# eora-ai/torchok

Measured on AMD Instinct MI355X. Metric: images/sec (node) ResNet-50 224px bs256/GPU; step p50 ms, higher is better.
Workload: dtype bf16

## Files before the change

torchok_amd/csrc/gemm256.hip:

```cpp
#include "conv_common.h"
#include <stdlib.h>

namespace {

typedef __attribute__((address_space(3))) void lds_void;
typedef __attribute__((address_space(3))) char lds_char;

constexpr int GT = 256;
constexpr int GK = 64;
constexpr int TILE_B = GT * GK * 2;
constexpr int STAGE_B = 2 * TILE_B;
constexpr int NBLK = STAGE_B / 1024;
constexpr int NI = NBLK / 8;

__device__ __forceinline__ u32x4 lds_read16(uint32_t addr) {
  u32x4 v;
  asm volatile("ds_read_b128 %0, %1" : "=v"(v) : "v"(addr));
  return v;
}
__device__ __forceinline__ float row16_sum_f(float v) {
  v += __builtin_bit_cast(float, __builtin_amdgcn_update_dpp(0, __builtin_bit_cast(int, v), 0x128, 0xF, 0xF, false));
  v += __builtin_bit_cast(float, __builtin_amdgcn_update_dpp(0, __builtin_bit_cast(int, v), 0x124, 0xF, 0xF, false));
  v += __builtin_bit_cast(float, __builtin_amdgcn_update_dpp(0, __builtin_bit_cast(int, v), 0x122, 0xF, 0xF, false));
  v += __builtin_bit_cast(float, __builtin_amdgcn_update_dpp(0, __builtin_bit_cast(int, v), 0x121, 0xF, 0xF, false));
  return v;
}

template <int MODE>
__global__ __launch_bounds__(512, 1) void gemm256_kernel(ConvArgs a) {
  extern __shared__ __attribute__((aligned(16))) char smem[];
  const uint32_t lds_base = (uint32_t)(size_t)(lds_char*)smem;
  const int tid = threadIdx.x;
  const int lane = tid & 63;
  const int wave = __builtin_amdgcn_readfirstlane(tid >> 6);
  const int r = lane & 15, g = lane >> 4;
  const int wn = wave & 1, wm = wave >> 1;

  const int ntiles = a.gridM * a.gridN;
  const int KD = a.Ktot;
  const int KT = (KD + GK - 1) / GK;

  const __amdgpu_buffer_rsrc_t xsrd = __builtin_amdgcn_make_buffer_rsrc((void*)a.x, 0, a.x_bytes, 0x00020000);
  const __amdgpu_buffer_rsrc_t wsrd = __builtin_amdgcn_make_buffer_rsrc((void*)a.w, 0, a.w_bytes, 0x00020000);

  uint32_t voff[NI];
  int kq[NI];
#pragma unroll
  for (int j = 0; j < NI; ++j) {
    const int row = ((j * 8 + wave) & 31) * 8 + (lane >> 3);
    kq[j] = ((lane & 7) ^ ((row & 3) | (((row >> 3) & 1) << 2))) * 8;
  }
  auto setup = [&](int id, int& m0, int& n0) {
    const int mt = id / a.gridN, nt = id - mt * a.gridN;
    m0 = mt * GT;
    n0 = nt * GT;
#pragma unroll
    for (int j = 0; j < NI; ++j) {
      const int bid = j * 8 + wave;
      const int row = (bid & 31) * 8 + (lane >> 3);
      const bool isw = bid < 32;
      const int grow = (isw ? n0 : m0) + row;
      const bool ok = grow < (isw ? a.K : a.M);
      voff[j] = ok ? (uint32_t)(((long long)grow * KD + kq[j]) * 2) : 0xFFFFFFF0u;
    }
  };
  auto issue = [&](int kt, int buf, bool live) {
#pragma unroll
    for (int j = 0; j < NI; ++j) {
      const int bid = j * 8 + wave;
      uint32_t off = (live && voff[j] != 0xFFFFFFF0u && kt * GK + kq[j] < KD) ? voff[j] + (uint32_t)(kt * (GK * 2)) : 0xFFFFFFF0u;
      asm volatile("" : "+v"(off));
      lds_void* dst = (lds_void*)(smem + buf * STAGE_B + bid * 1024);
      if (bid < 32) __builtin_amdgcn_raw_ptr_buffer_load_lds(wsrd, dst, 16, off, 0, 0, 0);
      else __builtin_amdgcn_raw_ptr_buffer_load_lds(xsrd, dst, 16, off, 0, 0, 0);
    }
  };

  const uint32_t swz = (uint32_t)((r & 3) | (((r >> 2) & 1) << 2));
  const uint32_t swx = (uint32_t)((r & 3) | (((r >> 3) & 1) << 2));
  const uint32_t a_lane = (uint32_t)((wn * 128 + 8 * (r >> 2) + (r & 3)) * 128);
  const uint32_t b_lane = (uint32_t)(TILE_B + (wm * 64 + r) * 128);
  uint32_t a_ch[2], b_ch[2];
#pragma unroll
  for (int kk = 0; kk < 2; ++kk) {
    a_ch[kk] = (((uint32_t)(4 * kk + g)) ^ swz) << 4;
    b_ch[kk] = (((uint32_t)(4 * kk + g)) ^ swx) << 4;
  }

  int tile = tok_xcd_remap(blockIdx.x, gridDim.x);
  int m0, n0;
  setup(tile, m0, n0);
  int base = 0;
  issue(0, base, tile < ntiles);
  while (tile < ntiles) {
  f32x4 acc[4][2][4];
#pragma unroll
  for (int p = 0; p < 4; ++p)
#pragma unroll
    for (int b = 0; b < 2; ++b)
#pragma unroll
      for (int mb = 0; mb < 4; ++mb) acc[p][b][mb] = (f32x4){0.f, 0.f, 0.f, 0.f};
  for (int kt = 0; kt < KT; ++kt) {
    const int buf = (base + kt) & 1;
    asm volatile("s_waitcnt vmcnt(0)" ::: "memory");
    __builtin_amdgcn_s_barrier();
    issue(kt + 1, buf ^ 1, kt + 1 < KT);
    const uint32_t sb = lds_base + (uint32_t)(buf * STAGE_B);
#pragma unroll
    for (int kk = 0; kk < 2; ++kk) {
      u32x4 af[4][2], bfr[4];
#pragma unroll
      for (int mb = 0; mb < 4; ++mb) bfr[mb] = lds_read16(sb + b_lane + (uint32_t)(mb * 16 * 128) + b_ch[kk]);
#pragma unroll
      for (int p = 0; p < 4; ++p)
#pragma unroll
        for (int b = 0; b < 2; ++b) af[p][b] = lds_read16(sb + a_lane + (uint32_t)((32 * p + 4 * b) * 128) + a_ch[kk]);
      asm volatile("s_waitcnt lgkmcnt(0)" ::: "memory");
      __builtin_amdgcn_sched_barrier(0);
#pragma unroll
      for (int p = 0; p < 4; ++p)
#pragma unroll
        for (int b = 0; b < 2; ++b)
#pragma unroll
          for (int mb = 0; mb < 4; ++mb)
            acc[p][b][mb] = __builtin_amdgcn_mfma_f32_16x16x32_bf16(__builtin_bit_cast(bf16x8, af[p][b]),
                                                                    __builtin_bit_cast(bf16x8, bfr[mb]), acc[p][b][mb], 0, 0, 0);
    }
  }
  const int cm0 = m0, cn0 = n0, cmt = m0 / GT;
  const int next = tile + gridDim.x;
  base = (base + KT) & 1;
  if (next < ntiles) {
    setup(next, m0, n0);
    issue(0, base, true);
  }

  float s1[4][8], s2[4][8];
  if constexpr (MODE >= 1 && MODE <= 3) {
#pragma unroll
    for (int p = 0; p < 4; ++p)
#pragma unroll
      for (int e = 0; e < 8; ++e) { s1[p][e] = 0.f; s2[p][e] = 0.f; }
  }
#pragma unroll
  for (int p = 0; p < 4; ++p) {
    const int n8 = cn0 + wn * 128 + 32 * p + 8 * g;
    const bool nok = n8 + 8 <= a.K;
    float bv[8];
#pragma unroll
    for (int e = 0; e < 8; ++e) bv[e] = (a.bias != nullptr && nok) ? a.bias[n8 + e] : 0.f;
#pragma unroll
    for (int mb = 0; mb < 4; ++mb) {
      const int pix = cm0 + wm * 64 + 16 * mb + r;
      if (pix < a.M && nok) {
        const size_t off = (size_t)pix * a.K + n8;
        float v[8];
#pragma unroll
        for (int e = 0; e < 8; ++e) v[e] = acc[p][e >> 2][mb][e & 3] + bv[e];
        if (a.accumulate) {
          const bf16x8 old = ldg16(a.y + off);
#pragma unroll
          for (int e = 0; e < 8; ++e) v[e] += bf2f(old[e]);
        }
        bf16x8 o;
#pragma unroll
        for (int e = 0; e < 8; ++e) o[e] = f2bf(v[e]);
        if constexpr (MODE == 3) {
          const unsigned bits = (unsigned)a.bn_mask[off >> 3];
#pragma unroll
          for (int e = 0; e < 8; ++e) {
            if (!((bits >> e) & 1u)) o[e] = (bf16)0.f;
            s1[p][e] += bf2f(o[e]);
          }
        }
        stg16(a.y + off, o);
        if constexpr (MODE == 1) {
#pragma unroll
          for (int e = 0; e < 8; ++e) {
            const float q = bf2f(o[e]);
            s1[p][e] += q;
            s2[p][e] = fmaf(q, q, s2[p][e]);
          }
        }
        if constexpr (MODE == 2) {
          const bf16x8 yv = ldg16(a.bn_y + off);
          const unsigned bits = a.bn_mask != nullptr ? (unsigned)a.bn_mask[off >> 3] : 0xffu;
#pragma unroll
          for (int e = 0; e < 8; ++e) {
            const float dz = ((bits >> e) & 1u) ? bf2f(o[e]) : 0.f;
            s1[p][e] += dz;
            s2[p][e] = fmaf(dz, bf2f(yv[e]), s2[p][e]);
          }
        }
      }
    }
  }
  if constexpr (MODE >= 1 && MODE <= 3) {
    float* red = reinterpret_cast<float*>(smem + 2 * STAGE_B);
#pragma unroll
    for (int p = 0; p < 4; ++p)
#pragma unroll
      for (int e = 0; e < 8; ++e) {
        const float t1 = row16_sum_f(s1[p][e]), t2 = row16_sum_f(s2[p][e]);
        if (r == 15) {
          const int nl = wn * 128 + 32 * p + 8 * g + e;
          red[(0 * 4 + wm) * GT + nl] = t1;
          red[(1 * 4 + wm) * GT + nl] = t2;
        }
      }
    asm volatile("s_waitcnt lgkmcnt(0)" ::: "memory");
    __builtin_amdgcn_s_barrier();
    const int which = tid >> 8, c = tid & 255;
    const float t = red[(which * 4 + 0) * GT + c] + red[(which * 4 + 1) * GT + c] + red[(which * 4 + 2) * GT + c] +
                    red[(which * 4 + 3) * GT + c];
    const int n = cn0 + c;
    if (n < a.K) a.stats[((size_t)which * a.stat_rows + cmt) * a.K + n] = t;
    if (cmt == a.gridM - 1 && n < a.K)
      for (int rr = a.gridM; rr < a.stat_rows; ++rr) a.stats[((size_t)which * a.stat_rows + rr) * a.K + n] = 0.f;
    asm volatile("s_waitcnt lgkmcnt(0)" ::: "memory");
    __builtin_amdgcn_s_barrier();
  }
  tile = next;
  }
  asm volatile("s_waitcnt vmcnt(0) lgkmcnt(0)" ::: "memory");
}

int g256_flag() {
  static const int v = [] { const char* e = getenv("TOK_GEMM256"); return (int)(e ? atoi(e) : 1); }();
  return v;
}
int g256_min_k() {
  static const int v = [] { const char* e = getenv("TOK_GEMM256_MIN_K"); return (int)(e ? atoi(e) : 256); }();
  return v;
}
int g256_min_tiles() {
  static const int v = [] { const char* e = getenv("TOK_GEMM256_MIN_TILES"); return (int)(e ? atoi(e) : 128); }();
  return v;
}

}

bool gemm256_modes(const ConvArgs& a) {
  if (a.ep_scale != nullptr || a.sub != nullptr) return false;
  if (a.mask_store && (a.bn_mask == nullptr || a.stats == nullptr)) return false;
  if (a.y2 != nullptr || a.act_x != nullptr) return false;
  return true;
}
bool gemm256_serves(const ConvArgs& a) { return gemm256_geometry(a) && gemm256_modes(a); }

bool gemm256_geometry(const ConvArgs& a) {
  const int flag = g256_flag();
  if (!flag) return false;
  if (!(a.R == 1 && a.S == 1 && a.stride == 1 && a.pad == 0 && a.C != 4)) return false;
  if (a.Ktot % 8 != 0 || a.K % 8 != 0 || a.Ktot <= GK) return false;
  if (flag >= 3) return true;
  if (a.K < 192 || a.M < 4096) return false;
  const long long tiles = (long long)tok_cdiv(a.M, GT) * tok_cdiv(a.K, GT);
  const int nt = tok_cdiv(a.K, GT);
  if ((long long)nt * GT * 3 > (long long)a.K * 4) return false;
  if (tiles < g256_min_tiles()) return false;
  if (flag >= 2) return a.Ktot >= g256_min_k();
  return a.Ktot >= 384;
}

int gemm256_rows(const ConvArgs& a) { return (tok_cdiv(a.M, GT) + 7) / 8 * 8; }

void gemm256_tiles(const ConvArgs& a, int* gridM, int* gridN) { *gridM = tok_cdiv(a.M, GT); *gridN = tok_cdiv(a.K, GT); }
int gemm256_grid(int gridM, int gridN) { return gridM * gridN < 256 ? gridM * gridN : 256; }

int gemm256_launch(ConvArgs& a, hipStream_t st) {
  constexpr int smem = 2 * STAGE_B + 2 * 4 * GT * 4;
  const int grid = a.grid;
  if (a.mask_store) tok_launch_lds<&gemm256_kernel<3>>(smem, dim3(grid), dim3(512), smem, st, a);
  else if (a.stats == nullptr) tok_launch_lds<&gemm256_kernel<0>>(smem, dim3(grid), dim3(512), smem, st, a);
  else if (a.bn_y == nullptr) tok_launch_lds<&gemm256_kernel<1>>(smem, dim3(grid), dim3(512), smem, st, a);
  else tok_launch_lds<&gemm256_kernel<2>>(smem, dim3(grid), dim3(512), smem, st, a);
  return 0;
}
```

Before: 14520.

## Prefetch epilogue loads in groups and specialize accumulate path at compile time

Restructures the GEMM epilogue so the residual, bn_y and mask loads for a group of output column strips are issued ahead of time and overlap with the math and stores of the previous group. Rows and columns past the edge are clamped rather than branched on, so the loads and stores stay uniform. Bias is folded into the accumulators up front, and accumulate becomes a template parameter, which doubles the number of kernel instantiations. The prefetch buffers raise register pressure, which may spill at one wave per SIMD.

```diff
diff --git a/torchok_amd/csrc/gemm256.hip b/torchok_amd/csrc/gemm256.hip
--- a/torchok_amd/csrc/gemm256.hip
+++ b/torchok_amd/csrc/gemm256.hip
@@ -1,5 +1,6 @@
 #include "conv_common.h"
 #include <stdlib.h>
+#include <type_traits>
 
 namespace {
 
@@ -26,7 +27,7 @@
   return v;
 }
 
-template <int MODE>
+template <int MODE, bool ACC>
 __global__ __launch_bounds__(512, 1) void gemm256_kernel(ConvArgs a) {
   extern __shared__ __attribute__((aligned(16))) char smem[];
   const uint32_t lds_base = (uint32_t)(size_t)(lds_char*)smem;
@@ -142,57 +143,133 @@
 #pragma unroll
       for (int e = 0; e < 8; ++e) { s1[p][e] = 0.f; s2[p][e] = 0.f; }
   }
+  constexpr bool PRE_Y = MODE == 2, PRE_BITS = MODE == 2 || MODE == 3;
+  constexpr bool want_old = ACC;
+  const bool want_bits = PRE_BITS && (MODE == 3 || a.bn_mask != nullptr);
+  const bool want_bias = a.bias != nullptr;
+  const int strip0 = cm0 + wm * 64, cbase = cn0 + wn * 128;
+  const int strip0c = strip0 < a.M ? strip0 : a.M - 1;
+  const size_t sbase = (size_t)strip0c * a.K;
+  bf16* const yb = a.y + sbase;
+  const bf16* const bnb = a.bn_y + sbase;
+  const uint8_t* const mkb = a.bn_mask + (sbase >> 3);
+  uint32_t erow[4], ecol[4];
+  bool rok[4], nok[4];
+#pragma unroll
+  for (int mb = 0; mb < 4; ++mb) {
+    const int rr = 16 * mb + r, last = a.M - 1 - strip0c;
+    rok[mb] = strip0 + rr < a.M;
+    erow[mb] = (uint32_t)((rr < last ? rr : last) * a.K);
+  }
 #pragma unroll
   for (int p = 0; p < 4; ++p) {
-    const int n8 = cn0 + wn * 128 + 32 * p + 8 * g;
-    const bool nok = n8 + 8 <= a.K;
-    float bv[8];
-#pragma unroll
-    for (int e = 0; e < 8; ++e) bv[e] = (a.bias != nullptr && nok) ? a.bias[n8 + e] : 0.f;
-#pragma unroll
-    for (int mb = 0; mb < 4; ++mb) {
-      const int pix = cm0 + wm * 64 + 16 * mb + r;
-      if (pix < a.M && nok) {
-        const size_t off = (size_t)pix * a.K + n8;
+    const int n8 = cbase + 32 * p + 8 * g;
+    nok[p] = n8 + 8 <= a.K;
+    ecol[p] = (uint32_t)(nok[p] ? n8 : a.K - 8);
+  }
+  constexpr int PG = (MODE == 2 && ACC) ? 1 : 2, NG = 4 / PG;
+  constexpr bool waits = PRE_Y || PRE_BITS || want_old;
+  bf16x8 pre_old[NG][PG][4], pre_y[NG][PG][4];
+  unsigned pre_bits[NG][PG][4];
+  auto request = [&](int gi) {
+#pragma unroll
+    for (int pp = 0; pp < PG; ++pp) {
+      const int p = PG * gi + pp;
+      if constexpr (want_old) {
+#pragma unroll
+        for (int mb = 0; mb < 4; ++mb) pre_old[gi][pp][mb] = ldg16(yb + (size_t)(erow[mb] + ecol[p]));
+      }
+      if constexpr (PRE_Y) {
+#pragma unroll
+        for (int mb = 0; mb < 4; ++mb) pre_y[gi][pp][mb] = ldg16(bnb + (size_t)(erow[mb] + ecol[p]));
+      }
+      if constexpr (PRE_BITS) {
+#pragma unroll
+        for (int mb = 0; mb < 4; ++mb) pre_bits[gi][pp][mb] = want_bits ? (unsigned)mkb[(size_t)((erow[mb] + ecol[p]) >> 3)] : 0xffu;
+      }
+    }
+  };
+  if (want_bias) {
+    float bv[4][8];
+#pragma unroll
+    for (int p = 0; p < 4; ++p)
+#pragma unroll
+      for (int e = 0; e < 8; ++e) bv[p][e] = a.bias[ecol[p] + e];
+#pragma unroll
+    for (int p = 0; p < 4; ++p)
+#pragma unroll
+      for (int mb = 0; mb < 4; ++mb)
+#pragma unroll
+        for (int e = 0; e < 8; ++e) acc[p][e >> 2][mb][e & 3] += bv[p][e];
+  }
+  request(0);
+#pragma unroll
+  for (int gi = 0; gi < NG; ++gi) {
+    if constexpr (waits) asm volatile("s_waitcnt vmcnt(0)" ::: "memory");
+    bf16x8 o[PG][4];
+#pragma unroll
+    for (int pp = 0; pp < PG; ++pp) {
+      const int p = PG * gi + pp;
+#pragma unroll
+      for (int mb = 0; mb < 4; ++mb) {
+        __builtin_amdgcn_sched_barrier(0);
+        const bool ok = rok[mb] && nok[p];
         float v[8];
 #pragma unroll
-        for (int e = 0; e < 8; ++e) v[e] = acc[p][e >> 2][mb][e & 3] + bv[e];
-        if (a.accumulate) {
-          const bf16x8 old = ldg16(a.y + off);
-#pragma unroll
-          for (int e = 0; e < 8; ++e) v[e] += bf2f(old[e]);
-        }
-        bf16x8 o;
-#pragma unroll
-        for (int e = 0; e < 8; ++e) o[e] = f2bf(v[e]);
+        for (int e = 0; e < 8; ++e) v[e] = acc[p][e >> 2][mb][e & 3];
+        if constexpr (want_old) {
+#pragma unroll
+          for (int e = 0; e < 8; ++e) v[e] += bf2f(pre_old[gi][pp][mb][e]);
+        }
+        bf16x8 q;
+#pragma unroll
+        for (int e = 0; e < 8; ++e) q[e] = f2bf(v[e]);
+        if (!ok) q = zero8();
         if constexpr (MODE == 3) {
-          const unsigned bits = (unsigned)a.bn_mask[off >> 3];
+          const unsigned bits = pre_bits[gi][pp][mb];
 #pragma unroll
           for (int e = 0; e < 8; ++e) {
-            if (!((bits >> e) & 1u)) o[e] = (bf16)0.f;
-            s1[p][e] += bf2f(o[e]);
+            if (!((bits >> e) & 1u)) q[e] = (bf16)0.f;
+            s1[p][e] += bf2f(q[e]);
           }
         }
-        stg16(a.y + off, o);
         if constexpr (MODE == 1) {
 #pragma unroll
           for (int e = 0; e < 8; ++e) {
-            const float q = bf2f(o[e]);
-            s1[p][e] += q;
-            s2[p][e] = fmaf(q, q, s2[p][e]);
+            const float t = bf2f(q[e]);
+            s1[p][e] += t;
+            s2[p][e] = fmaf(t, t, s2[p][e]);
           }
         }
         if constexpr (MODE == 2) {
-          const bf16x8 yv = ldg16(a.bn_y + off);
-          const unsigned bits = a.bn_mask != nullptr ? (unsigned)a.bn_mask[off >> 3] : 0xffu;
+          const unsigned bits = pre_bits[gi][pp][mb];
+          const bf16x8 yv = ok ? pre_y[gi][pp][mb] : zero8();
 #pragma unroll
           for (int e = 0; e < 8; ++e) {
-            const float dz = ((bits >> e) & 1u) ? bf2f(o[e]) : 0.f;
+            const float dz = ((bits >> e) & 1u) ? bf2f(q[e]) : 0.f;
             s1[p][e] += dz;
             s2[p][e] = fmaf(dz, bf2f(yv[e]), s2[p][e]);
           }
         }
-      }
+        o[pp][mb] = q;
+      }
+      if constexpr (MODE >= 1 && MODE <= 3) {
+#pragma unroll
+        for (int e = 0; e < 8; ++e) {
+          asm volatile("" : "+v"(s1[p][e]));
+          if constexpr (MODE != 3) asm volatile("" : "+v"(s2[p][e]));
+        }
+      }
+    }
+    __builtin_amdgcn_sched_barrier(0);
+    if (gi + 1 < NG) request(gi + 1);
+    __builtin_amdgcn_sched_barrier(0);
+#pragma unroll
+    for (int pp = 0; pp < PG; ++pp) {
+      const int p = PG * gi + pp;
+#pragma unroll
+      for (int mb = 0; mb < 4; ++mb)
+        if (rok[mb] && nok[p]) stg16(yb + (size_t)(erow[mb] + ecol[p]), o[pp][mb]);
     }
   }
   if constexpr (MODE >= 1 && MODE <= 3) {
@@ -271,9 +348,15 @@
 int gemm256_launch(ConvArgs& a, hipStream_t st) {
   constexpr int smem = 2 * STAGE_B + 2 * 4 * GT * 4;
   const int grid = a.grid;
-  if (a.mask_store) tok_launch_lds<&gemm256_kernel<3>>(smem, dim3(grid), dim3(512), smem, st, a);
-  else if (a.stats == nullptr) tok_launch_lds<&gemm256_kernel<0>>(smem, dim3(grid), dim3(512), smem, st, a);
-  else if (a.bn_y == nullptr) tok_launch_lds<&gemm256_kernel<1>>(smem, dim3(grid), dim3(512), smem, st, a);
-  else tok_launch_lds<&gemm256_kernel<2>>(smem, dim3(grid), dim3(512), smem, st, a);
+  const int mode = a.mask_store ? 3 : a.stats == nullptr ? 0 : a.bn_y == nullptr ? 1 : 2;
+  auto go = [&](auto acc) {
+    constexpr bool ACC = decltype(acc)::value;
+    if (mode == 3) tok_launch_lds<&gemm256_kernel<3, ACC>>(smem, dim3(grid), dim3(512), smem, st, a);
+    else if (mode == 0) tok_launch_lds<&gemm256_kernel<0, ACC>>(smem, dim3(grid), dim3(512), smem, st, a);
+    else if (mode == 1) tok_launch_lds<&gemm256_kernel<1, ACC>>(smem, dim3(grid), dim3(512), smem, st, a);
+    else tok_launch_lds<&gemm256_kernel<2, ACC>>(smem, dim3(grid), dim3(512), smem, st, a);
+  };
+  if (a.accumulate) go(std::true_type{});
+  else go(std::false_type{});
   return 0;
 }
```

Result: no change. 14560, median of 6 (+0.3%).
